# AvishaiBarnoy/genomics-lm

Measured on AMD Instinct MI355X. Metric: codon tokens/sec training step, 12L8H d512 seq1024, higher is better.
Workload: dtype bf16; 1 GPU; TinyGPT 12L8H d512 T1024 V68 train step; model=TinyGPT (genomics-lm src/codonlm), global_batch=32, seq_len=1024, micro_batch_per_gpu=32, parallelism=dp1, sep_mask=True

## Files before the change

genomics-lm_amd/codonlm_amd/ops.py:

```python
from __future__ import annotations

import ctypes as C

import torch

from . import _lib as L

_DT = {torch.float32: L.CG_F32, torch.bfloat16: L.CG_BF16}


def _dt(t: torch.Tensor) -> int:
    if t.dtype not in _DT:
        raise ValueError(f"unsupported dtype {t.dtype}")
    return _DT[t.dtype]


def _p(t):
    return None if t is None else t.data_ptr()


def gemm(a, b, *, a_kcontig=True, b_kcontig=True, M=None, N=None, K=None, out=None, out_dtype=None,
         bias=None, resid=None, epilogue=0, aux=None, aux_out=None, alpha=1.0, drop_seed=0, drop_p=0.0,
         split_k=1, colsum_out=None, n_valid=0, rope=None, tile=0, max_wg=0):
    for t in (a, b):
# ... 309 lines not shown
                               int(drop_seed) & 0xFFFFFFFF, float(drop_p), L.stream_ptr(tok_emb.device)),
            "cg_embed_fwd")
    return out


def attn_decode(q, cache, pos, H, KV, hd, segstate=None, window=0, Tmax=None):
    L.require_device(q, "attn_decode")
    L.require_device(cache, "attn_decode")
    if q.dtype != cache.dtype or cache.dim() != 3 or cache.stride(2) != 1 or q.stride(1) != 1:
        raise ValueError("attn_decode: q and cache share a dtype; cache is [B][Tmax][ldc]")
    B = q.shape[0]
    if Tmax is None:
        Tmax = cache.shape[1]
    if cache.shape[0] != B or cache.stride(0) != Tmax * cache.stride(1):
        raise ValueError("attn_decode: cache rows of one sequence must be Tmax consecutive rows")
    y = torch.empty(B, H * hd, dtype=q.dtype, device=q.device)
    L.check(L.lib.cg_attn_decode(_dt(q), q.data_ptr(), q.stride(0), cache.data_ptr(), cache.stride(1), int(Tmax),
                                 int(pos), _p(segstate), int(window or 0), B, H, KV, hd, y.data_ptr(), y.stride(0),
                                 L.stream_ptr(q.device)), "cg_attn_decode")
    return y


def attn_decode_ragged(q, cache, pos, H, KV, hd, segstate=None, window=0, Tmax=None, out=None):
    L.require_device(q, "attn_decode_ragged")
    L.require_device(cache, "attn_decode_ragged")
    L.require_device(pos, "attn_decode_ragged")
    if q.dtype != cache.dtype or cache.dim() != 3 or cache.stride(2) != 1 or q.stride(1) != 1:
        raise ValueError("attn_decode_ragged: q and cache share a dtype; cache is [B][Tmax][ldc]")
    B = q.shape[0]
    if Tmax is None:
        Tmax = cache.shape[1]
    if cache.shape[0] != B or cache.stride(0) != Tmax * cache.stride(1):
        raise ValueError("attn_decode_ragged: cache rows of one sequence must be Tmax consecutive rows")
    if pos.dtype != torch.int32 or pos.numel() != B or not pos.is_contiguous():
        raise ValueError("attn_decode_ragged: pos is a contiguous int32 [B]")
    y = out if out is not None else torch.zeros(B, H * hd, dtype=q.dtype, device=q.device)
    L.check(L.lib.cg_attn_decode_ragged(_dt(q), q.data_ptr(), q.stride(0), cache.data_ptr(), cache.stride(1),
                                        int(Tmax), pos.data_ptr(), _p(segstate), int(window or 0), B, H, KV, hd,
                                        y.data_ptr(), y.stride(0), L.stream_ptr(q.device)), "cg_attn_decode_ragged")
    return y


def sample_step(params, logits, state, next_tok, out_ids, n_active=None, term_logits=None):
    for t in (logits, state, next_tok, out_ids):
        L.require_device(t, "sample_step")
    B = logits.shape[0]
    if (logits.dtype != torch.float32 or state.dtype != torch.int32 or tuple(state.shape) != (B, 8)
            or not state.is_contiguous() or next_tok.dtype != torch.int64 or out_ids.dtype != torch.int64):
        raise ValueError("sample_step: logits fp32 [B][V], state int32 [B][8], next_tok / out_ids int64")
    L.check(L.lib.cg_sample_step(C.byref(params), logits.data_ptr(), logits.stride(0), _p(term_logits),
                                 term_logits.stride(0) if term_logits is not None else 0, state.data_ptr(),
                                 next_tok.data_ptr(), out_ids.data_ptr(), out_ids.stride(0), _p(n_active), B,
                                 L.stream_ptr(logits.device)), "cg_sample_step")


def attn_probs(qkv, segstart, lse, B, T, H, KV, hd, window=0):
    L.require_device(qkv, "attn_probs")
    out = torch.empty(B, H, T, T, dtype=torch.float32, device=qkv.device)
    L.check(L.lib.cg_attn_probs(_dt(qkv), qkv.data_ptr(), qkv.stride(0), _p(segstart), lse.data_ptr(), out.data_ptr(),
                                B, T, H, KV, hd, int(window or 0), L.stream_ptr(qkv.device)), "cg_attn_probs")
    return out


def segstate_step(tok, sep_id, pos, segstate):
    L.require_device(tok, "segstate_step")
    if tok.dtype != torch.int64 or segstate.dtype != torch.int32 or tok.numel() != segstate.numel():
        raise ValueError("segstate_step: int64 tokens [B], int32 state [B]")
    L.check(L.lib.cg_segstate_step(tok.contiguous().data_ptr(), tok.numel(), -1 if sep_id is None else int(sep_id),
                                   int(pos), segstate.data_ptr(), L.stream_ptr(tok.device)), "cg_segstate_step")
    return segstate


def _ids(values):
    vals = [int(v) for v in values]
    return (C.c_int * max(1, len(vals)))(*vals), len(vals)


def offset_targets(y, offset, boundary_ids=(2, 3), count=True):
    L.require_device(y, "offset_targets")
    y = y.to(torch.int64).contiguous()
    B, T = y.shape
    out = torch.empty_like(y)
    nv = torch.zeros((), dtype=torch.int32, device=y.device) if count else None
    ids, n = _ids(boundary_ids)
    L.check(L.lib.cg_offset_targets(y.data_ptr(), B, T, int(offset), ids, n, out.data_ptr(), _p(nv),
                                    L.stream_ptr(y.device)), "cg_offset_targets")
    return out, nv


def termination_labels(y, stop_ids, bucket_edges=(0, 3, 10, 30), ignore_index=-100):
    L.require_device(y, "termination_labels")
    y = y.to(torch.int64).contiguous()
    B, T = y.shape
    out = torch.empty_like(y)
    st, ns = _ids(stop_ids)
    ed, ne = _ids(bucket_edges)
    L.check(L.lib.cg_termination_labels(y.data_ptr(), B, T, st, ns, ed, ne, int(ignore_index), out.data_ptr(),
                                        L.stream_ptr(y.device)), "cg_termination_labels")
    return out


POOL_MODES = {"mean_nonpad": 0, "mean_content": 1, "eos": 2}


def pool_hidden(hidden, idx, mode, content_ids=(), pad_id=0):
    L.require_device(hidden, "pool_hidden")
    B, T, d = hidden.shape
    if hidden.stride(2) != 1 or hidden.stride(0) != T * hidden.stride(1):
        hidden = hidden.contiguous()
    idx = idx.to(device=hidden.device, dtype=torch.int64).contiguous()
    words = [0] * 8
    for t in content_ids:
        t = int(t)
        if not 0 <= t < 256:
            raise ValueError("content ids must be in [0, 256)")
        words[t >> 5] |= 1 << (t & 31)
    mask = (C.c_uint32 * 8)(*words)
    out = torch.empty(B, d, dtype=torch.float32, device=hidden.device)
    L.check(L.lib.cg_pool_hidden(_dt(hidden), hidden.data_ptr(), hidden.stride(1), idx.data_ptr(), B, T, d,
                                 int(pad_id), POOL_MODES[mode], mask, out.data_ptr(),
                                 L.stream_ptr(hidden.device)), "cg_pool_hidden")
    return out


def colsum(x, out=None, accumulate=False):
    L.require_device(x, "colsum")
    rows, cols = x.shape
    if out is None:
        out = torch.empty(cols, dtype=torch.float32, device=x.device)
    ws = torch.empty(int(L.lib.cg_colsum_workspace(rows, cols)) // 4 + 1, dtype=torch.float32, device=x.device)
    L.check(L.lib.cg_colsum(_dt(x), x.data_ptr(), x.stride(0), rows, cols, out.data_ptr(), int(bool(accumulate)),
                            ws.data_ptr(), ws.numel() * 4, L.stream_ptr(x.device)), "cg_colsum")
    return out


def transpose16(mats):
    if len(mats) > L.TRANSPOSE_MAX:
        raise ValueError("too many matrices")
    tb = L.TransposeBatch()
    tb.n = len(mats)
    outs = []
    for i, m in enumerate(mats):
        if m.element_size() != 2 or m.dim() != 2 or m.stride(1) != 1:
            raise ValueError("transpose16 takes row-major 2-byte matrices")
        L.require_device(m, "transpose16")
        o = torch.empty(m.shape[1], m.shape[0], dtype=m.dtype, device=m.device)
        tb.items[i] = L.TransposeItem(m.data_ptr(), o.data_ptr(), m.stride(0), o.stride(0), m.shape[0], m.shape[1])
        outs.append(o)
    if mats:
        L.check(L.lib.cg_transpose16_batch(C.byref(tb), L.stream_ptr(mats[0].device)), "cg_transpose16_batch")
    return outs


def gemm_dw_grouped(products, *, tile_m=0, ksplit=1):
    if not products:
        return
    if len(products) > L.DW_MAX:
        raise ValueError(f"at most {L.DW_MAX} products per group")
    g = L.DwGroup()
    g.n, g.tile_m = len(products), int(tile_m)
    K = None
    for i, (dy, x, out, alpha, acc, *cs) in enumerate(products):
        for t in (dy, x, out):
            L.require_device(t, "gemm_dw_grouped")
        if dy.dtype != torch.bfloat16 or x.dtype != torch.bfloat16 or out.dtype != torch.float32:
            raise ValueError("gemm_dw_grouped: bf16 operands, fp32 output")
        if K is None:
            K = dy.shape[0]
        if dy.shape[0] != K or x.shape[0] != K:
            raise ValueError("gemm_dw_grouped: every product reduces over the same K rows")
        p = g.p[i]
        p.A, p.lda, p.B, p.ldb = dy.data_ptr(), dy.stride(0), x.data_ptr(), x.stride(0)
        p.C, p.ldc = out.data_ptr(), out.stride(0)
        p.N_out, p.K_out = dy.shape[1], x.shape[1]
        if tuple(out.shape) != (p.N_out, p.K_out):
            raise ValueError("gemm_dw_grouped: out must be [N_out, K_out]")
        p.alpha, p.accumulate = float(alpha), int(bool(acc))
        if cs and cs[0] is not None:
            L.require_device(cs[0], "gemm_dw_grouped")
            if cs[0].dtype != torch.float32 or cs[0].numel() != p.N_out or not cs[0].is_contiguous():
                raise ValueError("gemm_dw_grouped: col_sum must be a contiguous fp32 [N_out]")
            p.col_sum = cs[0].data_ptr()
    g.K = int(K)
    ws = None
    if ksplit > 1:
        g.ksplit = int(ksplit)
        nbytes = int(L.lib.cg_gemm_dw_grouped_workspace(C.byref(g)))
        ws = torch.empty(max(nbytes, 16) // 4, dtype=torch.float32, device=products[0][0].device)
        g.workspace, g.ws_bytes = ws.data_ptr(), ws.numel() * 4
    L.check(L.lib.cg_gemm_dw_grouped(C.byref(g), L.stream_ptr(products[0][0].device)), "cg_gemm_dw_grouped")
    return ws
```

genomics-lm_amd/csrc/gemm.hip:

```cpp
#include "common.h"
#include <algorithm>

struct GemmParams {
  int M, N, K, kchunk;
  const void* A; long long lda;
  const void* B; long long ldb;
  void* C; long long ldc; int c_dtype;
  int epi; float alpha;
  const float* bias;
  const float* resid; long long ldr;
  const void* aux; void* aux_out; long long ld_aux;
  uint32_t drop_seed, drop_thr; float drop_scale;
  float* ws; int split;
  int n_valid;
  const float* rope_cos; const float* rope_sin;
  int rope_T, rope_half, rope_G, rope_mul, rope_uqk;
};

__device__ __forceinline__ void epi_apply(const GemmParams& p, int row, int col, float v) {
  const int e = p.epi;
  if (e & CG_EPI_BIAS) v += p.bias[col];
  const long long ai = (long long)row * p.ld_aux + col;
  if (e & CG_EPI_GELU) {
    const float s = (e & CG_EPI_GELU_DERIV) ? dgelu_f(v) : v;
// ... 667 lines not shown
  hipStream_t s = (hipStream_t)stream;
  GemmParams p{};
  p.M = d->M; p.N = d->N; p.K = d->K;
  p.A = d->A; p.lda = d->lda; p.B = d->B; p.ldb = d->ldb;
  p.C = d->C; p.ldc = d->ldc; p.c_dtype = d->c_dtype;
  p.epi = d->epilogue; p.alpha = d->alpha;
  p.bias = d->bias; p.resid = d->resid; p.ldr = d->ldr;
  p.aux = d->aux; p.aux_out = d->aux_out; p.ld_aux = d->ld_aux;
  p.drop_seed = d->drop_seed;
  p.drop_thr = cg_drop_threshold(d->drop_p);
  p.drop_scale = d->drop_p < 1.f ? 1.0f / (1.0f - d->drop_p) : 0.f;
  if ((p.epi & CG_EPI_ACCUM) && p.c_dtype != CG_F32) return CG_EINVAL;
  if ((p.epi & CG_EPI_BIAS) && !p.bias) return CG_EINVAL;
  if ((p.epi & CG_EPI_RESID) && !p.resid) return CG_EINVAL;
  if ((p.epi & CG_EPI_GELU) && !p.aux_out) return CG_EINVAL;
  if ((p.epi & CG_EPI_DGELU) && !p.aux) return CG_EINVAL;
  if ((p.epi & CG_EPI_GELU_DERIV) && !(p.epi & (CG_EPI_GELU | CG_EPI_DGELU))) return CG_EINVAL;
  if ((p.epi & CG_EPI_COLSUM) && (!d->workspace || d->split_k > 1)) return CG_EINVAL;
  if ((p.epi & CG_EPI_COLSUM) && d->ws_bytes < (size_t)cg_cdiv(p.M, 64) * (size_t)p.N * sizeof(float)) return CG_EINVAL;
  const bool swg = (p.epi & (CG_EPI_SWIGLU | CG_EPI_DSWIGLU)) != 0;
  if (swg) {
    if (p.epi != CG_EPI_SWIGLU && p.epi != CG_EPI_DSWIGLU) return CG_EUNSUPPORTED;
    if (d->in_dtype != CG_BF16 || p.c_dtype != CG_BF16 || d->split_k > 1 || !d->a_kcontig || !d->b_kcontig ||
        p.alpha != 1.0f || (p.N & 63) || (p.ldc & 7) || (p.ld_aux & 7) || ((uintptr_t)p.C & 15) ||
        ((uintptr_t)(p.epi == CG_EPI_SWIGLU ? p.aux_out : p.aux) & 15))
      return CG_EUNSUPPORTED;
    if (p.epi == CG_EPI_SWIGLU ? !p.aux_out : !p.aux) return CG_EINVAL;
    p.n_valid = d->n_valid > 0 ? std::min(d->n_valid, p.N) : p.N;
  }
  const bool rope = (p.epi & CG_EPI_ROPE) != 0;
  if (rope) {
    if ((p.epi & ~(CG_EPI_ROPE | CG_EPI_BIAS)) || !d->rope_cos || !d->rope_sin || d->rope_T <= 0) return CG_EINVAL;
    const int hd = d->rope_hd;
    if (d->in_dtype != CG_BF16 || p.c_dtype != CG_BF16 || d->split_k > 1 || hd <= 0 || hd % 16 ||
        d->rope_heads <= 0 || (long long)d->rope_heads * hd > p.N || p.N % 16 || p.N >= 65536 ||
        (((uintptr_t)d->rope_cos | (uintptr_t)d->rope_sin) & 15))
      return CG_EUNSUPPORTED;
    p.rope_cos = d->rope_cos;
    p.rope_sin = d->rope_sin;
    p.rope_T = d->rope_T;
    p.rope_half = hd / 2;
    p.rope_G = hd / 16;
    p.rope_mul = (65536 + p.rope_G - 1) / p.rope_G;
    p.rope_uqk = d->rope_heads * hd / 16;
  }
  if (d->tile < CG_TILE_AUTO || d->tile > CG_TILE_PERS_LW) return CG_EINVAL;
  if (d->tile != CG_TILE_AUTO && d->in_dtype != CG_BF16) return CG_EUNSUPPORTED;
  int split = d->split_k > 1 ? d->split_k : 1;
  const int bkt = d->in_dtype == CG_BF16 ? bfg::BKT : 16;
  if (d->K == 0) split = 1;
  int kchunk = cg_cdiv(cg_cdiv(d->K > 0 ? d->K : 1, split), bkt) * bkt;
  split = cg_cdiv(d->K > 0 ? d->K : 1, kchunk);
  if (split > 1 && (!d->workspace || d->ws_bytes < (size_t)split * (size_t)p.M * (size_t)p.N * sizeof(float)))
    return CG_EINVAL;
  p.kchunk = kchunk; p.split = split; p.ws = d->workspace;
  bool vec = false;
  const bool colsum = (p.epi & CG_EPI_COLSUM) != 0;
  bool colsum_fused = false;

  if (d->in_dtype == CG_F32) {
    p.epi &= ~CG_EPI_COLSUM;
    const bool big = !(d->lda & 3) && !(d->ldb & 3) && !((uintptr_t)d->A & 15) &&
                     !((uintptr_t)d->B & 15) && ((d->a_kcontig || d->b_kcontig) ? !(d->K & 3) : true) &&
                     (d->a_kcontig || !(d->M & 3)) && (d->b_kcontig || !(d->N & 3));
    if (big) {
      launch4(gemm_f32_big_kernel<false, false>, gemm_f32_big_kernel<false, true>, gemm_f32_big_kernel<true, false>,
              gemm_f32_big_kernel<true, true>, d->a_kcontig, d->b_kcontig,
              dim3(cg_cdiv(p.N, f32b::BN), cg_cdiv(p.M, f32b::BM), split), dim3(256), 0, s, p);
    } else {
      dim3 g(cg_cdiv(p.N, 64), cg_cdiv(p.M, 64), split);
      launch4(gemm_f32_kernel<false, false>, gemm_f32_kernel<false, true>, gemm_f32_kernel<true, false>,
              gemm_f32_kernel<true, true>, d->a_kcontig, d->b_kcontig, g, dim3(256), 0, s, p);
    }
  } else if (d->in_dtype == CG_BF16) {
    if ((d->lda & 7) || (d->ldb & 7)) return CG_EUNSUPPORTED;
    if (((uintptr_t)d->A & 15) || ((uintptr_t)d->B & 15)) return CG_EUNSUPPORTED;
    if (d->a_kcontig ? (d->K & 7) : (d->M & 7)) return CG_EUNSUPPORTED;
    if (d->b_kcontig ? (d->K & 7) : (d->N & 7)) return CG_EUNSUPPORTED;
    dim3 g(cg_cdiv(p.N, bfg::BN), cg_cdiv(p.M, bfg::BM), split);
    dim3 blk(256);
    size_t sh = bfg::SMEM;
    vec = vec_ok(d, split);
    gemm_kernel_t k;
    const bool pers = vec && use_pers(d, split);
    if ((swg || rope) && !pers) return CG_EUNSUPPORTED;
    if (!pers) p.epi &= ~CG_EPI_COLSUM;
    const int ke = split > 1 ? 0 : p.epi, kt = split > 1 ? CG_F32 : p.c_dtype;
    if (pers) {
      bool lw = false;
      k = pick_pers(p.epi, p.c_dtype, d->tile, &lw);
      colsum_fused = colsum;
      const int tiles = cg_cdiv(p.N, (p.epi & CG_EPI_SWIGLU) ? bfp::BN / 2 : bfp::BN) * cg_cdiv(p.M, bfp::BM);
      g = dim3(std::min(tiles, d->max_wg > 0 ? d->max_wg : cg_pers_cus()));
      blk = dim3(lw ? bfl::THREADS : bfp::THREADS);
      sh = lw ? bfl::SMEM : bfp::SMEM;
    } else if (vec && use_wide(d, kchunk, split)) {
      k = pick_spec<WideK>(d->a_kcontig, d->b_kcontig, ke, kt);
      g = dim3(cg_cdiv(p.N, bfw::BN) * cg_cdiv(p.M, bfw::BM) * split);
      blk = dim3(bfw::THREADS);
      sh = bfw::SMEM;
    } else if (vec && (d->tile == CG_TILE_AUTO || d->tile == CG_TILE_VEC)) {
      k = pick_spec<VecK>(d->a_kcontig, d->b_kcontig, ke, kt);
    } else if (d->tile != CG_TILE_AUTO && d->tile != CG_TILE_VEC) {
      return CG_EUNSUPPORTED;
    } else {
      k = d->a_kcontig ? (d->b_kcontig ? gemm_bf16_kernel<true, true> : gemm_bf16_kernel<true, false>)
                       : (d->b_kcontig ? gemm_bf16_kernel<false, true> : gemm_bf16_kernel<false, false>);
    }
    cg_func_lds((const void*)k, (int)sh);
    const int pk = pers ? CG_PROBE_GEMM_PERS
                        : d->a_kcontig ? (d->b_kcontig ? CG_PROBE_GEMM_FWD : CG_PROBE_GEMM_DX)
                                       : (d->b_kcontig ? CG_PROBE_NONE : CG_PROBE_GEMM_DW);
    cg_probe_begin(pk, s);
    hipLaunchKernelGGL(k, g, blk, sh, s, p);
    if (cg_probe_kind() == pk) {
      const double M = p.M, N = p.N, K = p.K, ce = p.c_dtype == CG_F32 ? 4.0 : 2.0;
      const bool sw = (p.epi & CG_EPI_SWIGLU) != 0, dsw = (p.epi & CG_EPI_DSWIGLU) != 0;
      const double nb = sw ? 2.0 * N : N;
      double bytes = 2.0 * (M * K + nb * K) + M * N * ce;
      if (p.epi & CG_EPI_BIAS) bytes += 4.0 * N;
      if (p.epi & CG_EPI_RESID) bytes += 4.0 * M * N;
      if (p.epi & (CG_EPI_GELU | CG_EPI_DGELU)) bytes += M * N * ce;
      if (p.epi & CG_EPI_ACCUM) bytes += 4.0 * M * N;
      if (sw) bytes += 2.0 * M * 2.0 * N;
      if (dsw) bytes += 2.0 * M * 2.0 * N + M * N * ce;
      if (p.epi & CG_EPI_COLSUM) bytes += 4.0 * cg_cdiv(p.M, 64) * N;
      cg_probe_end(pk, s, 2.0 * M * nb * K, bytes);
    }
  } else {
    return CG_EUNSUPPORTED;
  }
  CG_LAUNCH_CHECK();
  if (split > 1) {
    const long long total = (long long)p.M * p.N;
    if (vec) {
      int blocks = (int)((total / 8 + 255) / 256);
      if (blocks > 4096) blocks = 4096;
      hipLaunchKernelGGL(splitk_reduce_vec_kernel, dim3(blocks), dim3(256), 0, s, p);
    } else {
      int blocks = (int)((total + 255) / 256);
      if (blocks > 4096) blocks = 4096;
      hipLaunchKernelGGL(splitk_reduce_kernel, dim3(blocks), dim3(256), 0, s, p);
    }
    CG_LAUNCH_CHECK();
  }
  if (colsum && !colsum_fused) {
    hipLaunchKernelGGL(colsum64_kernel, dim3(cg_cdiv(p.N, 256), cg_cdiv(p.M, 64)), dim3(256), 0, s, p.C, p.ldc,
                       p.c_dtype, p.M, p.N, p.ws);
    CG_LAUNCH_CHECK();
  }
  return CG_OK;
}

static bool dw_tile_code(int bm) { return bm == 128 || bm == 129 || bm == 256 || bm == 512; }
extern "C" int cg_gemm_dw_tiles(int bm, int N_out, int K_out) {
  if (!dw_tile_code(bm)) bm = 128;
  return cg_cdiv(N_out, bm >= 256 ? 256 : 128) * cg_cdiv(K_out, bm == 512 ? 256 : 128);
}
template <int BM, int NS, int BNT = bfd::BN>
static int launch_dw(bfd::Params& P, hipStream_t s) {
  using G = bfd::Geo<BM, NS, BNT>;
  bool cs = false;
  for (int i = 0; i < P.nprod; ++i) cs |= P.p[i].colsum != nullptr;
  auto kern = cs ? gemm_dw_kernel<BM, NS, BNT, true> : gemm_dw_kernel<BM, NS, BNT, false>;
  int ntiles = 0;
  for (int i = 0; i < P.nprod; ++i) {
    bfd::Prod& pr = P.p[i];
    pr.tiles_n = cg_cdiv(pr.K_out, BNT);
    pr.tile0 = ntiles;
    ntiles += cg_cdiv(pr.N_out, BM) * pr.tiles_n;
  }
  P.ntiles = ntiles * P.ksplit;
  if (!ntiles) return CG_OK;
  if (P.ksplit > 1) P.kc_steps = cg_cdiv(cg_cdiv(P.K, P.ksplit), bfd::BKT);
  const int grid = std::min(P.ntiles, P.max_wg > 0 ? P.max_wg : cg_pers_cus());
  cg_func_lds((const void*)kern, G::SMEM);
  double flops = 0, bytes = 0;
  for (int i = 0; i < P.nprod; ++i) {
    const bfd::Prod& q = P.p[i];
    flops += 2.0 * q.N_out * (double)q.K_out * P.K;
    bytes += 2.0 * P.K * ((double)q.N_out + q.K_out) + (q.accum ? 8.0 : 4.0) * q.N_out * (double)q.K_out;
  }
  cg_probe_begin(CG_PROBE_GEMM_DW_GROUPED, s);
  hipLaunchKernelGGL(kern, dim3(grid), dim3(G::THREADS), G::SMEM, s, P);
  cg_probe_end(CG_PROBE_GEMM_DW_GROUPED, s, flops, bytes);
  if (P.ksplit > 1) {
    long long most = 0;
    double elems = 0;
    for (int i = 0; i < P.nprod; ++i) {
      most = std::max<long long>(most, (long long)P.p[i].N_out * P.p[i].K_out / 4);
      elems += (double)P.p[i].N_out * P.p[i].K_out;
    }
    cg_probe_begin(CG_PROBE_DW_SLAB, s);
    hipLaunchKernelGGL(dw_slab_reduce_kernel, dim3((unsigned)std::min<long long>(cg_cdiv(most, 256), 512), P.nprod),
                       dim3(256), 0, s, P);
    cg_probe_end(CG_PROBE_DW_SLAB, s, (P.ksplit - 1) * elems, (4.0 * (P.ksplit - 1) + 8.0) * elems);
  }
  CG_LAUNCH_CHECK();
  return CG_OK;
}
extern "C" size_t cg_gemm_dw_grouped_workspace(const cg_dw_group* grp) {
  if (!grp || grp->ksplit <= 1) return 0;
  size_t e = 0;
  for (int i = 0; i < grp->n && i < CG_DW_MAX; ++i)
    if (grp->p[i].N_out > 0 && grp->p[i].K_out > 0) e += (size_t)grp->p[i].N_out * (size_t)grp->p[i].K_out;
  return (size_t)(grp->ksplit - 1) * e * sizeof(float);
}
extern "C" size_t cg_gemm_dw_grouped_workspace(const cg_dw_group* grp);
extern "C" int cg_gemm_dw_grouped(const cg_dw_group* grp, void* stream) {
  if (!grp || grp->n < 0 || grp->n > CG_DW_MAX || grp->K <= 0) return CG_EINVAL;
  bfd::Params P{};
  P.nprod = 0;
  P.K = grp->K;
  const long long lim = (1ll << 31) - (1ll << 24);
  for (int i = 0; i < grp->n; ++i) {
    const cg_dw_product& q = grp->p[i];
    if (q.N_out <= 0 || q.K_out <= 0) continue;
    if (!q.A || !q.B || !q.C) return CG_EINVAL;
    if (q.N_out % 8 || q.K_out % 8 || q.lda % 8 || q.ldb % 8 || q.ldc % 4 || q.lda < q.N_out || q.ldb < q.K_out ||
        q.ldc < q.K_out)
      return CG_EUNSUPPORTED;
    if (((uintptr_t)q.A & 15) || ((uintptr_t)q.B & 15) || ((uintptr_t)q.C & 15)) return CG_EUNSUPPORTED;
    if (((long long)(grp->K - 1) * q.lda + q.N_out) * 2 >= lim || ((long long)(grp->K - 1) * q.ldb + q.K_out) * 2 >= lim)
      return CG_EUNSUPPORTED;
    bfd::Prod& pr = P.p[P.nprod++];
    pr.A = (const bf16_t*)q.A; pr.lda = q.lda;
    pr.B = (const bf16_t*)q.B; pr.ldb = q.ldb;
    pr.C = q.C; pr.ldc = q.ldc;
    pr.N_out = q.N_out; pr.K_out = q.K_out;
    pr.alpha = q.alpha; pr.accum = q.accumulate;
    pr.colsum = q.col_sum;
    if (q.col_sum && grp->ksplit > 1) return CG_EUNSUPPORTED;
  }
  if (!P.nprod) return CG_OK;
  P.ksplit = grp->ksplit > 1 ? grp->ksplit : 1;
  if (P.ksplit > 8) return CG_EUNSUPPORTED;
  if (P.ksplit > 1) {
    if (!grp->workspace || ((uintptr_t)grp->workspace & 15) || grp->ws_bytes < cg_gemm_dw_grouped_workspace(grp))
      return CG_EINVAL;
    P.slab = grp->workspace;
    long long off = 0;
    for (int i = 0; i < P.nprod; ++i) {
      P.slab_off[i] = off;
      off += (long long)P.p[i].N_out * P.p[i].K_out;
    }
    P.slab_stride = off;
  }
  hipStream_t s = (hipStream_t)stream;
  const int bm = grp->tile_m > 0 ? grp->tile_m : 128;
  P.max_wg = grp->max_wg;
  if (bm == 512) return launch_dw<256, 2, 256>(P, s);
  if (bm == 256) return launch_dw<256, 3>(P, s);
  if (bm == 129) return launch_dw<128, 5>(P, s);
  return launch_dw<128, 4>(P, s);
}
```

genomics-lm_amd/csrc/gemm_dw.h:

```cpp
namespace bfd {
constexpr int BN = 128, BKT = 64;

__device__ __forceinline__ void dma16_asm(__amdgpu_buffer_rsrc_t r, uint32_t lds, uint32_t voff) {
  uint32_t keep;
  asm volatile(
      "s_mov_b32 %0, m0\n\ts_mov_b32 m0, %2\n\ts_nop 0\n\tbuffer_load_dwordx4 %1, %3, 0 offen lds\n\t"
      "s_mov_b32 m0, %0"
      : "=&s"(keep)
      : "v"(voff), "s"(lds), "s"(r)
      : "memory");
}

template <int BM, int NSTAGE, int BNT = BN>
struct Geo {
  static constexpr int WAVES = BM / 32;
  static constexpr int JN = BNT / 32;
  static constexpr int THREADS = WAVES * 64;
  static constexpr int STAGES = NSTAGE;
  static constexpr int A_BYTES = BM * BKT * 2;
  static constexpr int B_BYTES = BNT * BKT * 2;
  static constexpr int STAGE_BYTES = A_BYTES + B_BYTES;
  static constexpr int A_CHUNKS = A_BYTES / 1024 / WAVES;
  static constexpr int B_CHUNKS = B_BYTES / 1024 / WAVES;
  static constexpr int DPS = A_CHUNKS + B_CHUNKS;
  static constexpr int SMEM = STAGES * STAGE_BYTES;
};

struct Prod {
  const bf16_t* A;
  const bf16_t* B;
  float* C;
  long long lda, ldb, ldc;
  int N_out, K_out, tiles_n, tile0;
  float alpha;
  int accum;
  float* colsum;
};
struct Params {
  Prod p[CG_DW_MAX];
  int nprod, K, ntiles;
  int ksplit, kc_steps;
  int max_wg;
  float* slab;
  long long slab_stride;
  long long slab_off[CG_DW_MAX];
};
}

template <int BM, int NSTAGE, int BNT, bool CS>
__global__ __launch_bounds__((bfd::Geo<BM, NSTAGE, BNT>::THREADS), 1) void gemm_dw_kernel(const bfd::Params P) {
  using namespace bfd;
  using G = Geo<BM, NSTAGE, BNT>;
  constexpr int JN = G::JN;
  constexpr int S = G::STAGES;
  extern __shared__ __attribute__((aligned(16))) char smem[];
  const int tid = threadIdx.x, lane = tid & 63;
  const int wave = __builtin_amdgcn_readfirstlane(tid >> 6);
  const uint32_t lds0 = (uint32_t)(uintptr_t)smem;
  const int nblk = gridDim.x;
  const int lb = cg_xcd_remap(blockIdx.x, nblk);
  const int my_tiles = lb < P.ntiles ? (P.ntiles - 1 - lb) / nblk + 1 : 0;
  const int nt = P.ksplit > 1 ? P.kc_steps : (P.K + BKT - 1) / BKT;
  const int wm = (wave >> 1) * 64, wn = (wave & 1) * (BNT / 2);
  if (my_tiles == 0) return;

  auto find = [&](int tile, int& pi) {
    pi = 0;
    while (pi + 1 < P.nprod && tile >= P.p[pi + 1].tile0) ++pi;
  };
  uint32_t va[G::A_CHUNKS], vb[G::B_CHUNKS];
  __amdgpu_buffer_rsrc_t ra, rb;
  uint32_t a_org = 0, b_org = 0, a_step = 0, b_step = 0;
  int dk = 0, dt = 0;
  auto load_tile = [&]() {
    if (dk >= my_tiles) {
      a_org = b_org = 0x80000000u;
      a_step = b_step = 0;
      return;
    }
    int pi;
    const int item = lb + dk * nblk;
    const int tile = item / P.ksplit, sl = item - tile * P.ksplit;
    find(tile, pi);
    const Prod& pr = P.p[pi];
    const int lt = tile - pr.tile0;
    const int m0 = (lt / pr.tiles_n) * BM, n0 = (lt % pr.tiles_n) * BNT;
    ra = __builtin_amdgcn_make_buffer_rsrc((void*)pr.A, (short)0,
                                           (int)(((long long)(P.K - 1) * pr.lda + pr.N_out) * 2), 0x00020000);
    rb = __builtin_amdgcn_make_buffer_rsrc((void*)pr.B, (short)0,
                                           (int)(((long long)(P.K - 1) * pr.ldb + pr.K_out) * 2), 0x00020000);
    const long long r0 = (long long)sl * nt * BKT;
    a_org = (uint32_t)((long long)m0 * 2 + r0 * pr.lda * 2);
    b_org = (uint32_t)((long long)n0 * 2 + r0 * pr.ldb * 2);
    a_step = (uint32_t)(BKT * pr.lda * 2);
    b_step = (uint32_t)(BKT * pr.ldb * 2);
#pragma unroll
    for (int i = 0; i < G::A_CHUNKS; ++i) va[i] = bfw::src_off<false>((wave + G::WAVES * i) * 1024 + 16 * lane, pr.lda);
#pragma unroll
    for (int i = 0; i < G::B_CHUNKS; ++i) vb[i] = bfw::src_off<false>((wave + G::WAVES * i) * 1024 + 16 * lane, pr.ldb);
  };
  auto advance = [&]() {
    if (++dt == nt) {
      dt = 0;
      ++dk;
      load_tile();
    }
  };
  auto issue = [&](int g) {
    const uint32_t st = __builtin_amdgcn_readfirstlane(lds0 + (g % S) * G::STAGE_BYTES + wave * 1024);
    const uint32_t ao = a_org + dt * a_step, bo = b_org + dt * b_step;
#pragma unroll
    for (int i = 0; i < G::A_CHUNKS; ++i) dma16_asm(ra, st + G::WAVES * i * 1024, ao + va[i]);
#pragma unroll
    for (int i = 0; i < G::B_CHUNKS; ++i) dma16_asm(rb, st + G::A_BYTES + G::WAVES * i * 1024, bo + vb[i]);
    advance();
  };

  v4f acc[4][JN];
  float cs[4];
  auto step = [&](int g, auto cs_c) __attribute__((always_inline)) {
    constexpr bool TCS = decltype(cs_c)::value;
    asm volatile("s_waitcnt vmcnt(%0)" ::"n"((S - 2) * G::DPS) : "memory");
    __builtin_amdgcn_s_barrier();
    const char* st = smem + (g % S) * G::STAGE_BYTES;
    const char* as = st + (wm >> 7) * 16384;
    const int ar = wm & 127;
    const char* bs = st + G::A_BYTES + (wn >> 7) * 16384;
    const int bc = wn & 127;
    v8bf af[2][4], bfr[2][JN];
#pragma unroll
    for (int i = 0; i < 4; ++i) af[0][i] = bfg::frag<false>(as, ar + 16 * i, 0, lane);
#pragma unroll
    for (int j = 0; j < JN; ++j) bfr[0][j] = bfg::frag<false>(bs, bc + 16 * j, 0, lane);
    const uint32_t nx = __builtin_amdgcn_readfirstlane(lds0 + ((g + S - 1) % S) * G::STAGE_BYTES + wave * 1024);
    const uint32_t ao = a_org + dt * a_step, bo = b_org + dt * b_step;
    if constexpr (JN == 4) {
#pragma unroll
      for (int gr = 0; gr < 8; ++gr) {
        const int i = gr >> 1, j0 = 2 * (gr & 1);
        acc[i][j0] = __builtin_amdgcn_mfma_f32_16x16x32_bf16(bfr[0][j0], af[0][i], acc[i][j0], 0, 0, 0);
        acc[i][j0 + 1] = __builtin_amdgcn_mfma_f32_16x16x32_bf16(bfr[0][j0 + 1], af[0][i], acc[i][j0 + 1], 0, 0, 0);
        if (gr < 4) af[1][gr] = bfg::frag<false>(as, ar + 16 * gr, 1, lane);
        else bfr[1][gr - 4] = bfg::frag<false>(bs, bc + 16 * (gr - 4), 1, lane);
        if (gr < G::A_CHUNKS) dma16_asm(ra, nx + G::WAVES * gr * 1024, ao + va[gr]);
        else if (gr < G::DPS) dma16_asm(rb, nx + G::A_BYTES + G::WAVES * (gr - G::A_CHUNKS) * 1024, bo + vb[gr - G::A_CHUNKS]);
      }
    } else {
#pragma unroll
      for (int j = 0; j < JN; ++j) {
#pragma unroll
        for (int i = 0; i < 4; ++i)
          acc[i][j] = __builtin_amdgcn_mfma_f32_16x16x32_bf16(bfr[0][j], af[0][i], acc[i][j], 0, 0, 0);
        bfr[1][j] = bfg::frag<false>(bs, bc + 16 * j, 1, lane);
        if (j < 4) af[1][j] = bfg::frag<false>(as, ar + 16 * j, 1, lane);
        if (j < G::A_CHUNKS) dma16_asm(ra, nx + G::WAVES * j * 1024, ao + va[j]);
        else if (j < G::DPS) dma16_asm(rb, nx + G::A_BYTES + G::WAVES * (j - G::A_CHUNKS) * 1024, bo + vb[j - G::A_CHUNKS]);
      }
    }
#pragma unroll
    for (int i = 0; i < 4; ++i)
#pragma unroll
      for (int j = 0; j < JN; ++j)
        acc[i][j] = __builtin_amdgcn_mfma_f32_16x16x32_bf16(bfr[1][j], af[1][i], acc[i][j], 0, 0, 0);
    if constexpr (JN == 4) {
      __builtin_amdgcn_sched_group_barrier(0x100, 16, 0);
#pragma unroll
      for (int gr = 0; gr < 8; ++gr) {
        __builtin_amdgcn_sched_group_barrier(0x008, 2, 0);
        __builtin_amdgcn_sched_group_barrier(0x100, 2, 0);
        if (gr < G::DPS) __builtin_amdgcn_sched_group_barrier(SGB_DMA, 1, 0);
      }
      __builtin_amdgcn_sched_group_barrier(0x008, 16, 0);
    } else {
      __builtin_amdgcn_sched_group_barrier(0x100, 2 * (4 + JN), 0);
#pragma unroll
      for (int j = 0; j < JN; ++j) {
        __builtin_amdgcn_sched_group_barrier(0x008, 4, 0);
        if (j < 4) __builtin_amdgcn_sched_group_barrier(0x100, 4, 0);
        else __builtin_amdgcn_sched_group_barrier(0x100, 2, 0);
        if (j < G::DPS) __builtin_amdgcn_sched_group_barrier(SGB_DMA, 1, 0);
      }
      __builtin_amdgcn_sched_group_barrier(0x008, 4 * JN, 0);
    }
    if constexpr (TCS) {
      typedef __bf16 bf2_t __attribute__((ext_vector_type(2)));
      const bf2_t one2 = __builtin_bit_cast(bf2_t, 0x3F803F80u);
#pragma unroll
      for (int h = 0; h < 2; ++h)
#pragma unroll
        for (int i = 0; i < 4; ++i) {
          const uint4 u = __builtin_bit_cast(uint4, af[h][i]);
          cs[i] = __builtin_amdgcn_fdot2_f32_bf16(__builtin_bit_cast(bf2_t, u.x), one2, cs[i], false);
          cs[i] = __builtin_amdgcn_fdot2_f32_bf16(__builtin_bit_cast(bf2_t, u.y), one2, cs[i], false);
          cs[i] = __builtin_amdgcn_fdot2_f32_bf16(__builtin_bit_cast(bf2_t, u.z), one2, cs[i], false);
          cs[i] = __builtin_amdgcn_fdot2_f32_bf16(__builtin_bit_cast(bf2_t, u.w), one2, cs[i], false);
        }
    }
    advance();
  };

  auto epilogue = [&](int k) {
    const int item = lb + k * nblk;
    const int tile = item / P.ksplit, sl = item - tile * P.ksplit;
    int pi;
    find(tile, pi);
    const Prod& pr = P.p[pi];
    const int lt = tile - pr.tile0;
    const int m0 = (lt / pr.tiles_n) * BM, n0 = (lt % pr.tiles_n) * BNT;
    const int g4 = lane >> 4, r16 = lane & 15;
    if (sl > 0) {
      float* slab = P.slab + (long long)(sl - 1) * P.slab_stride + P.slab_off[pi];
#pragma unroll
      for (int i = 0; i < 4; ++i) {
        const int m = m0 + wm + 16 * i + r16;
#pragma unroll
        for (int j = 0; j < JN; ++j) {
          const int n = n0 + wn + 16 * j + 4 * g4;
          if (m < pr.N_out && n < pr.K_out)
            *(float4*)(slab + (long long)m * pr.K_out + n) =
                make_float4(acc[i][j][0] * pr.alpha, acc[i][j][1] * pr.alpha, acc[i][j][2] * pr.alpha,
                            acc[i][j][3] * pr.alpha);
        }
      }
      return;
    }
#pragma unroll
    for (int i = 0; i < 4; ++i) {
      const int m = m0 + wm + 16 * i + r16;
#pragma unroll
      for (int j = 0; j < JN; ++j) {
        const int n = n0 + wn + 16 * j + 4 * g4;
        if (m < pr.N_out && n < pr.K_out) {
          float4* c = (float4*)(pr.C + (long long)m * pr.ldc + n);
          float4 v = make_float4(acc[i][j][0] * pr.alpha, acc[i][j][1] * pr.alpha, acc[i][j][2] * pr.alpha,
                                 acc[i][j][3] * pr.alpha);
          if (pr.accum) {
            const float4 o = *c;
            v.x += o.x; v.y += o.y; v.z += o.z; v.w += o.w;
          }
          *c = v;
        }
      }
    }
  };

  load_tile();
#pragma unroll
  for (int s = 0; s < S - 1; ++s) issue(s);
  int g = 0;
  for (int k = 0; k < my_tiles; ++k) {
#pragma unroll
    for (int i = 0; i < 4; ++i)
#pragma unroll
      for (int j = 0; j < JN; ++j) acc[i][j] = (v4f){0.f, 0.f, 0.f, 0.f};
    int cpi = -1;
    if constexpr (CS) {
      const int tile = (lb + k * nblk) / P.ksplit;
      int pi;
      find(tile, pi);
      if (P.p[pi].colsum && (tile - P.p[pi].tile0) % P.p[pi].tiles_n == 0) cpi = pi;
    }
    if (cpi >= 0) {
#pragma unroll
      for (int i = 0; i < 4; ++i) cs[i] = 0.f;
      for (int t = 0; t < nt; ++t, ++g) step(g, std::true_type{});
      const Prod& pr = P.p[cpi];
      if (wn == 0) {
        const int m0 = ((lb + k * nblk) - pr.tile0) / pr.tiles_n * BM;
#pragma unroll
        for (int i = 0; i < 4; ++i) {
          float v = cs[i];
          v += __shfl_xor(v, 16);
          v += __shfl_xor(v, 32);
          const int m = m0 + wm + 16 * i + (lane & 15);
          if ((lane >> 4) == 0 && m < pr.N_out) pr.colsum[m] = v * pr.alpha + (pr.accum ? pr.colsum[m] : 0.f);
        }
      }
    } else {
      for (int t = 0; t < nt; ++t, ++g) step(g, std::false_type{});
    }
    epilogue(k);
  }
  asm volatile("s_waitcnt vmcnt(0)" ::: "memory");
}

__global__ __launch_bounds__(256) void dw_slab_reduce_kernel(const bfd::Params P) {
  const bfd::Prod& pr = P.p[blockIdx.y];
  const float* slab = P.slab + P.slab_off[blockIdx.y];
  const long long n4 = (long long)pr.N_out * pr.K_out / 4;
  for (long long e = blockIdx.x * 256ll + threadIdx.x; e < n4; e += (long long)gridDim.x * 256) {
    const long long idx = 4 * e;
    const int m = (int)(idx / pr.K_out), n = (int)(idx - (long long)m * pr.K_out);
    float4* c = (float4*)(pr.C + (long long)m * pr.ldc + n);
    float4 v = *c;
    for (int s = 1; s < P.ksplit; ++s) {
      const float4 w = *(const float4*)(slab + (long long)(s - 1) * P.slab_stride + idx);
      v.x += w.x; v.y += w.y; v.z += w.z; v.w += w.w;
    }
    *c = v;
  }
}
```

Baseline: 2.289 million tokens/s.

## Add 32-token ring-buffered stages with register double-buffering to 256x256 dW kernel

For the 512 tile code, the weight-gradient GEMM now uses 32-token K stages in a 5-slot LDS ring instead of two 64-token stages. A new step32 path double-buffers register fragments, reading the next stage's fragments and issuing DMA interleaved with the MFMAs under explicit sched_group_barrier hints. The aim is deeper prefetch and better overlap of LDS reads and global loads with matrix math. The Python wrapper also gains max_wg and a reusable workspace argument. This adds complexity, including colsum handling for every tile when CS is set, and only takes effect when callers pass tile_m=512.

```diff
diff --git a/genomics-lm_amd/codonlm_amd/ops.py b/genomics-lm_amd/codonlm_amd/ops.py
--- a/genomics-lm_amd/codonlm_amd/ops.py
+++ b/genomics-lm_amd/codonlm_amd/ops.py
@@ -485,13 +485,13 @@
     return outs
 
 
-def gemm_dw_grouped(products, *, tile_m=0, ksplit=1):
+def gemm_dw_grouped(products, *, tile_m=0, ksplit=1, max_wg=0, workspace=None):
     if not products:
         return
     if len(products) > L.DW_MAX:
         raise ValueError(f"at most {L.DW_MAX} products per group")
     g = L.DwGroup()
-    g.n, g.tile_m = len(products), int(tile_m)
+    g.n, g.tile_m, g.max_wg = len(products), int(tile_m), int(max_wg)
     K = None
     for i, (dy, x, out, alpha, acc, *cs) in enumerate(products):
         for t in (dy, x, out):
@@ -519,7 +519,13 @@
     if ksplit > 1:
         g.ksplit = int(ksplit)
         nbytes = int(L.lib.cg_gemm_dw_grouped_workspace(C.byref(g)))
-        ws = torch.empty(max(nbytes, 16) // 4, dtype=torch.float32, device=products[0][0].device)
+        ws = workspace
+        if ws is None:
+            ws = torch.empty(max(nbytes, 16) // 4, dtype=torch.float32, device=products[0][0].device)
+        elif ws.dtype != torch.float32 or not ws.is_contiguous() or ws.numel() * 4 < nbytes:
+            raise ValueError(f"gemm_dw_grouped: workspace must be contiguous fp32 of at least {nbytes} bytes")
+        else:
+            L.require_device(ws, "gemm_dw_grouped")
         g.workspace, g.ws_bytes = ws.data_ptr(), ws.numel() * 4
     L.check(L.lib.cg_gemm_dw_grouped(C.byref(g), L.stream_ptr(products[0][0].device)), "cg_gemm_dw_grouped")
     return ws
diff --git a/genomics-lm_amd/csrc/gemm.hip b/genomics-lm_amd/csrc/gemm.hip
--- a/genomics-lm_amd/csrc/gemm.hip
+++ b/genomics-lm_amd/csrc/gemm.hip
@@ -843,17 +843,20 @@
   return CG_OK;
 }
 
+#ifndef DW_RING_SLOTS
+#define DW_RING_SLOTS 5
+#endif
 static bool dw_tile_code(int bm) { return bm == 128 || bm == 129 || bm == 256 || bm == 512; }
 extern "C" int cg_gemm_dw_tiles(int bm, int N_out, int K_out) {
   if (!dw_tile_code(bm)) bm = 128;
   return cg_cdiv(N_out, bm >= 256 ? 256 : 128) * cg_cdiv(K_out, bm == 512 ? 256 : 128);
 }
-template <int BM, int NS, int BNT = bfd::BN>
+template <int BM, int NS, int BNT = bfd::BN, int BKT = DW_KUNIT>
 static int launch_dw(bfd::Params& P, hipStream_t s) {
-  using G = bfd::Geo<BM, NS, BNT>;
+  using G = bfd::Geo<BM, NS, BNT, BKT>;
   bool cs = false;
   for (int i = 0; i < P.nprod; ++i) cs |= P.p[i].colsum != nullptr;
-  auto kern = cs ? gemm_dw_kernel<BM, NS, BNT, true> : gemm_dw_kernel<BM, NS, BNT, false>;
+  auto kern = cs ? gemm_dw_kernel<BM, NS, BNT, true, BKT> : gemm_dw_kernel<BM, NS, BNT, false, BKT>;
   int ntiles = 0;
   for (int i = 0; i < P.nprod; ++i) {
     bfd::Prod& pr = P.p[i];
@@ -863,7 +866,7 @@
   }
   P.ntiles = ntiles * P.ksplit;
   if (!ntiles) return CG_OK;
-  if (P.ksplit > 1) P.kc_steps = cg_cdiv(cg_cdiv(P.K, P.ksplit), bfd::BKT);
+  if (P.ksplit > 1) P.kc_steps = dw_kc_steps(P.K, P.ksplit);
   const int grid = std::min(P.ntiles, P.max_wg > 0 ? P.max_wg : cg_pers_cus());
   cg_func_lds((const void*)kern, G::SMEM);
   double flops = 0, bytes = 0;
@@ -940,7 +943,7 @@
   hipStream_t s = (hipStream_t)stream;
   const int bm = grp->tile_m > 0 ? grp->tile_m : 128;
   P.max_wg = grp->max_wg;
-  if (bm == 512) return launch_dw<256, 2, 256>(P, s);
+  if (bm == 512) return launch_dw<256, DW_RING_SLOTS, 256, 32>(P, s);
   if (bm == 256) return launch_dw<256, 3>(P, s);
   if (bm == 129) return launch_dw<128, 5>(P, s);
   return launch_dw<128, 4>(P, s);
diff --git a/genomics-lm_amd/csrc/gemm_dw.h b/genomics-lm_amd/csrc/gemm_dw.h
--- a/genomics-lm_amd/csrc/gemm_dw.h
+++ b/genomics-lm_amd/csrc/gemm_dw.h
@@ -1,5 +1,6 @@
+#include "gemm_dw_ring.h"
 namespace bfd {
-constexpr int BN = 128, BKT = 64;
+constexpr int BN = 128;
 
 __device__ __forceinline__ void dma16_asm(__amdgpu_buffer_rsrc_t r, uint32_t lds, uint32_t voff) {
   uint32_t keep;
@@ -11,8 +12,11 @@
       : "memory");
 }
 
-template <int BM, int NSTAGE, int BNT = BN>
+template <int BM, int NSTAGE, int BNT = BN, int BKT_ = DW_KUNIT>
 struct Geo {
+  static constexpr int BKT = BKT_;
+  static constexpr int SPU = DW_KUNIT / BKT;
+  static constexpr int SUB_BYTES = BKT * 256;
   static constexpr int WAVES = BM / 32;
   static constexpr int JN = BNT / 32;
   static constexpr int THREADS = WAVES * 64;
@@ -47,20 +51,23 @@
 };
 }
 
-template <int BM, int NSTAGE, int BNT, bool CS>
-__global__ __launch_bounds__((bfd::Geo<BM, NSTAGE, BNT>::THREADS), 1) void gemm_dw_kernel(const bfd::Params P) {
+template <int BM, int NSTAGE, int BNT, bool CS, int BKT = DW_KUNIT>
+__global__ __launch_bounds__((bfd::Geo<BM, NSTAGE, BNT, BKT>::THREADS), 1) void gemm_dw_kernel(const bfd::Params P) {
   using namespace bfd;
-  using G = Geo<BM, NSTAGE, BNT>;
+  using G = Geo<BM, NSTAGE, BNT, BKT>;
   constexpr int JN = G::JN;
   constexpr int S = G::STAGES;
-  extern __shared__ __attribute__((aligned(16))) char smem[];
+  constexpr int SPU = G::SPU;
+  static_assert(BKT == 64 || (BKT == 32 && JN == 8 && S >= 4 && G::A_CHUNKS <= 4 && G::DPS <= 8),
+                "32-token stages: 256 x 256 tile only");
+  extern __shared__ __attribute__((aligned(256))) char smem[];
   const int tid = threadIdx.x, lane = tid & 63;
   const int wave = __builtin_amdgcn_readfirstlane(tid >> 6);
   const uint32_t lds0 = (uint32_t)(uintptr_t)smem;
   const int nblk = gridDim.x;
   const int lb = cg_xcd_remap(blockIdx.x, nblk);
   const int my_tiles = lb < P.ntiles ? (P.ntiles - 1 - lb) / nblk + 1 : 0;
-  const int nt = P.ksplit > 1 ? P.kc_steps : (P.K + BKT - 1) / BKT;
+  const int nt = dw_units(P.K, P.ksplit, P.kc_steps);
   const int wm = (wave >> 1) * 64, wn = (wave & 1) * (BNT / 2);
   if (my_tiles == 0) return;
 
@@ -89,25 +96,25 @@
                                            (int)(((long long)(P.K - 1) * pr.lda + pr.N_out) * 2), 0x00020000);
     rb = __builtin_amdgcn_make_buffer_rsrc((void*)pr.B, (short)0,
                                            (int)(((long long)(P.K - 1) * pr.ldb + pr.K_out) * 2), 0x00020000);
-    const long long r0 = (long long)sl * nt * BKT;
+    const long long r0 = dw_stage_row0(sl, nt, 0, BKT);
     a_org = (uint32_t)((long long)m0 * 2 + r0 * pr.lda * 2);
     b_org = (uint32_t)((long long)n0 * 2 + r0 * pr.ldb * 2);
     a_step = (uint32_t)(BKT * pr.lda * 2);
     b_step = (uint32_t)(BKT * pr.ldb * 2);
 #pragma unroll
-    for (int i = 0; i < G::A_CHUNKS; ++i) va[i] = bfw::src_off<false>((wave + G::WAVES * i) * 1024 + 16 * lane, pr.lda);
-#pragma unroll
-    for (int i = 0; i < G::B_CHUNKS; ++i) vb[i] = bfw::src_off<false>((wave + G::WAVES * i) * 1024 + 16 * lane, pr.ldb);
+    for (int i = 0; i < G::A_CHUNKS; ++i) va[i] = dw_src_off((wave + G::WAVES * i) * 1024 + 16 * lane, pr.lda, BKT);
+#pragma unroll
+    for (int i = 0; i < G::B_CHUNKS; ++i) vb[i] = dw_src_off((wave + G::WAVES * i) * 1024 + 16 * lane, pr.ldb, BKT);
   };
   auto advance = [&]() {
-    if (++dt == nt) {
+    if (++dt == nt * SPU) {
       dt = 0;
       ++dk;
       load_tile();
     }
   };
   auto issue = [&](int g) {
-    const uint32_t st = __builtin_amdgcn_readfirstlane(lds0 + (g % S) * G::STAGE_BYTES + wave * 1024);
+    const uint32_t st = __builtin_amdgcn_readfirstlane(lds0 + dw_slot(g, S) * G::STAGE_BYTES + wave * 1024);
     const uint32_t ao = a_org + dt * a_step, bo = b_org + dt * b_step;
 #pragma unroll
     for (int i = 0; i < G::A_CHUNKS; ++i) dma16_asm(ra, st + G::WAVES * i * 1024, ao + va[i]);
@@ -123,9 +130,9 @@
     asm volatile("s_waitcnt vmcnt(%0)" ::"n"((S - 2) * G::DPS) : "memory");
     __builtin_amdgcn_s_barrier();
     const char* st = smem + (g % S) * G::STAGE_BYTES;
-    const char* as = st + (wm >> 7) * 16384;
+    const char* as = st + (wm >> 7) * G::SUB_BYTES;
     const int ar = wm & 127;
-    const char* bs = st + G::A_BYTES + (wn >> 7) * 16384;
+    const char* bs = st + G::A_BYTES + (wn >> 7) * G::SUB_BYTES;
     const int bc = wn & 127;
     v8bf af[2][4], bfr[2][JN];
 #pragma unroll
@@ -197,6 +204,79 @@
         }
     }
     advance();
+  };
+
+  v8bf af[2][4], bfr[2][JN];
+  const uint32_t fl0 = dw_frag_lane_off(lane, 0), fl1 = dw_frag_lane_off(lane, 1);
+  auto frag32 = [&](uint32_t img, int rr0) {
+    typedef v4s __attribute__((address_space(3))) * lp4;
+    const v4s lo = __builtin_amdgcn_ds_read_tr16_b64_v4i16((lp4)(uintptr_t)dw_frag_addr(img, fl0, rr0));
+    const v4s hi = __builtin_amdgcn_ds_read_tr16_b64_v4i16((lp4)(uintptr_t)dw_frag_addr(img, fl1, rr0));
+    const v8s r = {lo[0], lo[1], lo[2], lo[3], hi[0], hi[1], hi[2], hi[3]};
+    return __builtin_bit_cast(v8bf, r);
+  };
+  const uint32_t a_img = lds0 + (wm >> 7) * G::SUB_BYTES, b_img = lds0 + G::A_BYTES + (wn >> 7) * G::SUB_BYTES;
+  const int ar = wm & 127, bc = wn & 127;
+  auto read_first = [&]() {
+    asm volatile("s_waitcnt vmcnt(%0)" ::"n"(dw_wait_count(S, G::DPS, false)) : "memory");
+    __builtin_amdgcn_s_barrier();
+#pragma unroll
+    for (int i = 0; i < 4; ++i) af[0][i] = frag32(a_img, ar + 16 * i);
+#pragma unroll
+    for (int j = 0; j < JN; ++j) bfr[0][j] = frag32(b_img, bc + 16 * j);
+  };
+  auto step32 = [&](int g, auto cur_c, auto cs_c) __attribute__((always_inline)) {
+    constexpr int CUR = decltype(cur_c)::value, NXT = CUR ^ 1;
+    constexpr bool TCS = decltype(cs_c)::value;
+    if constexpr (TCS) {
+      typedef __bf16 bf2_t __attribute__((ext_vector_type(2)));
+      const bf2_t one2 = __builtin_bit_cast(bf2_t, 0x3F803F80u);
+#pragma unroll
+      for (int i = 0; i < 4; ++i) {
+        const uint4 u = __builtin_bit_cast(uint4, af[CUR][i]);
+        cs[i] = __builtin_amdgcn_fdot2_f32_bf16(__builtin_bit_cast(bf2_t, u.x), one2, cs[i], false);
+        cs[i] = __builtin_amdgcn_fdot2_f32_bf16(__builtin_bit_cast(bf2_t, u.y), one2, cs[i], false);
+        cs[i] = __builtin_amdgcn_fdot2_f32_bf16(__builtin_bit_cast(bf2_t, u.z), one2, cs[i], false);
+        cs[i] = __builtin_amdgcn_fdot2_f32_bf16(__builtin_bit_cast(bf2_t, u.w), one2, cs[i], false);
+        asm volatile("" : "+v"(cs[i]));
+      }
+    }
+    asm volatile("s_waitcnt vmcnt(%0)" ::"n"(dw_wait_count(S, G::DPS, true)) : "memory");
+    __builtin_amdgcn_s_barrier();
+    const uint32_t st = dw_slot(g + 1, S) * G::STAGE_BYTES;
+    const uint32_t as = a_img + st, bs = b_img + st;
+    const uint32_t nx =
+        __builtin_amdgcn_readfirstlane(lds0 + dw_slot(dw_issue_stage(g, S), S) * G::STAGE_BYTES + wave * 1024);
+    const uint32_t ao = a_org + dt * a_step, bo = b_org + dt * b_step;
+#pragma unroll
+    for (int j = 0; j < JN; ++j) {
+#pragma unroll
+      for (int i = 0; i < 4; ++i)
+        acc[i][j] = __builtin_amdgcn_mfma_f32_16x16x32_bf16(bfr[CUR][j], af[CUR][i], acc[i][j], 0, 0, 0);
+      bfr[NXT][j] = frag32(bs, bc + 16 * j);
+      if (j < 4) af[NXT][j] = frag32(as, ar + 16 * j);
+      if (j < G::A_CHUNKS) dma16_asm(ra, nx + G::WAVES * j * 1024, ao + va[j]);
+      else if (j < G::DPS) dma16_asm(rb, nx + G::A_BYTES + G::WAVES * (j - G::A_CHUNKS) * 1024, bo + vb[j - G::A_CHUNKS]);
+    }
+#pragma unroll
+    for (int j = 0; j < JN; ++j) {
+      __builtin_amdgcn_sched_group_barrier(0x008, 4, 0);
+      if (j < 4) __builtin_amdgcn_sched_group_barrier(0x100, 4, 0);
+      else __builtin_amdgcn_sched_group_barrier(0x100, 2, 0);
+      if (j < G::DPS) __builtin_amdgcn_sched_group_barrier(SGB_DMA, 1, 0);
+    }
+    advance();
+  };
+  auto unit = [&](int& g, auto cs_c) __attribute__((always_inline)) {
+    if constexpr (BKT == 64) {
+      step(g, cs_c);
+      ++g;
+    } else {
+      step32(g, std::integral_constant<int, 0>{}, cs_c);
+      ++g;
+      step32(g, std::integral_constant<int, 1>{}, cs_c);
+      ++g;
+    }
   };
 
   auto epilogue = [&](int k) {
@@ -247,6 +327,7 @@
   load_tile();
 #pragma unroll
   for (int s = 0; s < S - 1; ++s) issue(s);
+  if constexpr (BKT == 32) read_first();
   int g = 0;
   for (int k = 0; k < my_tiles; ++k) {
 #pragma unroll
@@ -260,12 +341,12 @@
       find(tile, pi);
       if (P.p[pi].colsum && (tile - P.p[pi].tile0) % P.p[pi].tiles_n == 0) cpi = pi;
     }
-    if (cpi >= 0) {
+    if (cpi >= 0 || (CS && BKT == 32)) {
 #pragma unroll
       for (int i = 0; i < 4; ++i) cs[i] = 0.f;
-      for (int t = 0; t < nt; ++t, ++g) step(g, std::true_type{});
-      const Prod& pr = P.p[cpi];
-      if (wn == 0) {
+      for (int t = 0; t < nt; ++t) unit(g, std::true_type{});
+      const Prod& pr = P.p[cpi >= 0 ? cpi : 0];
+      if (wn == 0 && cpi >= 0) {
         const int m0 = ((lb + k * nblk) - pr.tile0) / pr.tiles_n * BM;
 #pragma unroll
         for (int i = 0; i < 4; ++i) {
@@ -277,7 +358,7 @@
         }
       }
     } else {
-      for (int t = 0; t < nt; ++t, ++g) step(g, std::false_type{});
+      for (int t = 0; t < nt; ++t) unit(g, std::false_type{});
     }
     epilogue(k);
   }
diff --git a/genomics-lm_amd/csrc/gemm_dw_ring.h b/genomics-lm_amd/csrc/gemm_dw_ring.h
--- /dev/null
+++ b/genomics-lm_amd/csrc/gemm_dw_ring.h
@@ -0,0 +1,35 @@
+#pragma once
+#if defined(__HIPCC__) || defined(__CUDACC__)
+#define DW_HD __host__ __device__ constexpr
+#else
+#define DW_HD constexpr
+#endif
+
+constexpr int DW_KUNIT = 64;
+
+DW_HD int dw_kc_steps(int K, int ksplit) {
+  const int per = (K + ksplit - 1) / ksplit;
+  return (per + DW_KUNIT - 1) / DW_KUNIT;
+}
+DW_HD int dw_units(int K, int ksplit, int kc_steps) { return ksplit > 1 ? kc_steps : (K + DW_KUNIT - 1) / DW_KUNIT; }
+DW_HD long long dw_stage_row0(int sl, int nt, int dt, int bkt) {
+  return (long long)sl * nt * DW_KUNIT + (long long)dt * bkt;
+}
+DW_HD int dw_slot(int g, int S) { return g % S; }
+DW_HD int dw_issue_stage(int g, int S) { return g + S - 1; }
+DW_HD int dw_wait_count(int S, int dps, bool read_ahead) { return (S - 2 - (read_ahead ? 1 : 0)) * dps; }
+
+DW_HD unsigned dw_src_off(int pos, long long ld, int bkt) {
+  const int sub_bytes = bkt * 256;
+  const int sub = pos / sub_bytes, q = pos % sub_bytes;
+  const int krow = q >> 8, phys = (q >> 4) & 15;
+  const int ch = phys ^ (((krow & 3) << 2) | ((krow >> 2) & 3));
+  return (unsigned)(((long long)krow * ld + 128 * sub + 8 * ch) * 2);
+}
+
+DW_HD unsigned dw_frag_lane_off(int lane, int hi) {
+  const int krow = 8 * (lane >> 4) + ((lane & 15) >> 2) + 4 * hi;
+  const int e = (lane & 3) >> 1;
+  return (unsigned)(krow * 256 + 16 * (e ^ (((krow & 3) << 2) | ((krow >> 2) & 3))) + 8 * (lane & 1));
+}
+DW_HD unsigned dw_frag_addr(unsigned img, unsigned lane_off, int rr0) { return (img + lane_off) ^ (unsigned)(2 * rr0); }
```

Measured after the change: 2.327 million tokens/s, median of 6. +1.6%, better.
